# antonilo/unsupervised_detection

Hardware: AMD Instinct MI355X
Metric: frame-pairs/sec per adversarial step, DAVIS 480p batch4, 1/2/4/8 GPU (higher is better)
Workload: dtype f32

## Files before the change

### include/udet_debug.h

```cpp
#ifndef UDET_DEBUG_H
#define UDET_DEBUG_H
#include <stddef.h>
#ifdef __cplusplus
extern "C" {
#endif
void udet_debug_force_conv(int bm, int bn, int ks);
void udet_debug_conv_fp16(int on);
void udet_debug_force_wgrad(int nsplit, int dma);
int udet_debug_last_wgrad(void);
int udet_debug_last_wgrad_reduce(void);
int udet_debug_conv2d_backward_filter_ex(const float* x, int ldx, int x_coff, const float* dy, int ldy, int y_coff, const float* y_saved, int act,
                                         float alpha, const float* w, const float* b, const float* gamma, float bn_c, float* dw, float* db,
                                         float* dgamma, float* dbeta, int n, int h, int wd, int cin, int cout, int k, int stride, int dilation,
                                         int up, void* workspace, size_t workspace_bytes, void* stream);
void udet_debug_upb_min_pixels(long v);
void udet_debug_set_tuning(int on);
void udet_debug_force_pair(int on);
int udet_debug_last_pair(void);
int udet_debug_conv2d_pair(const float* xa, const float* xb, const float* wa, const float* wb, const float* ba, const float* bb, float* ya, float* yb,
                           int na, int nb, int h, int w, int cin, int cout, int k, int stride, int dilation, int act, float alpha, void* workspace,
                           size_t workspace_bytes, void* stream);
int udet_debug_last_conv(void);
#ifdef __cplusplus
}
#endif
#endif
```

### unsupervised_detection_amd/_devel.py

```python
from __future__ import annotations

import ctypes
import os

from ._ffi import lib as _lib

_PATH = os.path.join(os.path.dirname(os.path.abspath(__file__)), "libudet_debug.so")
if not os.path.exists(_PATH):
    raise RuntimeError(f"{_PATH} is missing: build it with `make -C unsupervised_detection_amd/csrc`")
dbg = ctypes.CDLL(_PATH, mode=ctypes.RTLD_GLOBAL)
dbg.udet_debug_force_conv.restype = None
dbg.udet_debug_force_conv.argtypes = [ctypes.c_int, ctypes.c_int, ctypes.c_int]
dbg.udet_debug_last_conv.restype = ctypes.c_int
dbg.udet_debug_last_conv.argtypes = []
dbg.udet_debug_conv_fp16.restype = None
dbg.udet_debug_conv_fp16.argtypes = [ctypes.c_int]
dbg.udet_debug_force_wgrad.restype = None
dbg.udet_debug_force_wgrad.argtypes = [ctypes.c_int, ctypes.c_int]
dbg.udet_debug_upb_min_pixels.restype = None
dbg.udet_debug_upb_min_pixels.argtypes = [ctypes.c_long]
dbg.udet_debug_set_tuning.restype = None
dbg.udet_debug_set_tuning.argtypes = [ctypes.c_int]
dbg.udet_debug_last_wgrad.restype = ctypes.c_int
dbg.udet_debug_last_wgrad.argtypes = []
dbg.udet_debug_force_pair.restype = None
dbg.udet_debug_force_pair.argtypes = [ctypes.c_int]
dbg.udet_debug_last_pair.restype = ctypes.c_int
dbg.udet_debug_last_pair.argtypes = []
dbg.udet_debug_conv2d_pair.restype = ctypes.c_int
dbg.udet_debug_conv2d_pair.argtypes = [ctypes.c_void_p] * 8 + [ctypes.c_int] * 10 + [ctypes.c_float, ctypes.c_void_p, ctypes.c_size_t, ctypes.c_void_p]
dbg.udet_debug_last_wgrad_reduce.restype = ctypes.c_int
dbg.udet_debug_last_wgrad_reduce.argtypes = []
_p, _i, _f = ctypes.c_void_p, ctypes.c_int, ctypes.c_float
dbg.udet_debug_conv2d_backward_filter_ex.restype = ctypes.c_int
dbg.udet_debug_conv2d_backward_filter_ex.argtypes = ([_p, _i, _i, _p, _i, _i, _p, _i, _f, _p, _p, _p, _f, _p, _p, _p, _p] + [_i] * 9
                                                     + [_p, ctypes.c_size_t, _p])
```

### unsupervised_detection_amd/csrc/conv_host.h

```cpp
#pragma once
#include "common.h"
namespace udet {
void same_pad(int in, int k, int s, int d, int* before, int* out);
void conv_setup_fwd(ConvParams& p, int N, int H, int W, int kh, int kw, int s, int d);
int conv_dgrad_classes(int s, int H, int W);
void conv_force_config(int bm, int bn, int ks);
bool conv_thin_n_ok(const ConvParams& p);
bool conv_thin_k_ok(const ConvParams& p);
int launch_conv_thin_n(const ConvParams& p, hipStream_t stream);
int launch_conv_thin_k(const ConvParams& p, hipStream_t stream);
bool conv_wino_geometry(const ConvParams& p, int* dil, int widx_at[9]);
bool conv_wino_ok(const ConvParams& p);
bool conv_wino_variant_ok(const ConvParams& p, int variant);
int conv_wino_np(int cout);
size_t conv_wino_floats(int Kc, int cout);
long conv_wino_workgroups(const ConvParams& p, int variant);
int conv_wino_max_ksplit(const ConvParams& p, int variant);
int launch_conv_wino(ConvParams& p, int variant, int ks, hipStream_t stream);
int launch_splitk_second_pass(const ConvParams& p, hipStream_t stream);
int launch_wino_pack(const float* src, float* dst, int R, int C, int Kc, int np, int k_split, int k_gap, int transposed, hipStream_t stream);
int launch_wino_from_packed(const ConvParams& p, float* dst, int np, hipStream_t stream);
void conv_debug_f16(int on);
int conv_debug_f16_on();
int conv_last_config();
void conv_set_tuning(int on);
int tuned_shapes();
void tune_dump(FILE* f);
bool tune_put_line(const char* line);
int conv_tune_rejected();
void wgrad_set_tuning(int on);
bool wgrad_wino_ok(const WgradParams& p);
int wgrad_wino_slices(const WgradParams& p, int wanted);
int launch_wgrad_wino(const WgradParams& q, int slices, int ldn, hipStream_t stream);
int wgrad_last_config();
enum { WGRAD_RED_FUSED_BN = 1 << 26, WGRAD_RED_SEPARATE_BN = 1 << 27, WGRAD_RED_SWAPPED = 1 << 28, WGRAD_RED_CLASSES = 1 << 29 };
int wgrad_last_reduce();
void setup_up_fwd(ConvParams& p, int N, int H, int W);
void wgrad_force(int nsplit, int dma);
void conv_force_pair(int on);
int conv_last_pair();
#define UDET_TUNE_ABI 6
bool conv_setup_dgrad(ConvParams& p, int cls, int N, int H, int W, int kh, int kw, int s, int d);
int launch_pack_weights(const float* src, float* dst, int T, int R, int C, int Kc, int ldw, int k_split, int k_gap,
                        int mode, const float* scale, hipStream_t stream);
int launch_pack_taps_into_n(const float* src, float* dst, int T, int R, int C, int Kc, int ldz, int k_split, int k_gap,
                            int transposed, hipStream_t stream);
int launch_pack_jobs(const PackJob* jobs_dev, int njobs, const float* wsrc, float* ws, float bn_c, hipStream_t stream);
int launch_fold_bn(const float* b, const float* gamma, const float* beta, float c, float* scale, float* bias_f, int n,
                   hipStream_t stream);
int launch_copy_channels(const float* src, int lds, int s_coff, float* dst, int ldd, int d_coff, long P, int C, float mul,
                         float add, hipStream_t stream);
int launch_warp(const float* img, const float* flow, int ldf, int f_coff, float flow_scale, float* out, int N, int H,
                int W, int C, int* dbg_idx, float* dbg_alpha, hipStream_t stream);
int launch_cost_volume(const float* c1, const float* wr, float* out, int ldo, int o_coff, int N, int H, int W, int C,
                       hipStream_t stream);
int launch_warp_cost_volume(const float* c1, const float* c2, const float* flow, int ldf, int f_coff, float flow_scale, float* out,
                            int ldo, int corr_coff, int c1_coff, float* warped_dbg, int N, int H, int W, int C, hipStream_t stream);
inline int round_up(int v, int m) { return (v + m - 1) / m * m; }
}
```

### unsupervised_detection_amd/csrc/conv_tile.hip

```cpp
#include <type_traits>

#include "common.h"
#include "conv_epilogue.h"

namespace udet {

typedef float floatx16 __attribute__((ext_vector_type(16)));
typedef _Float16 halfx4 __attribute__((ext_vector_type(4)));

__device__ __forceinline__ void tile_epilogue(const ConvParams& p, int off, int n, float v) {
  if (p.bias) v += p.bias[n];
  v = act_fwd(v, p.act, p.alpha);
  if (p.y2) p.y2[(size_t)off * p.ldy2 + p.y2_coff + n] = v;
  if (p.res) v += p.res[(size_t)off * p.ldres + p.res_coff + n];
  float* dst = p.y + (size_t)off * p.ldy + p.y_coff + n;
  if (p.accumulate) v += *dst;
  *dst = v;
  if (p.uo && n >= p.u_c0 && n < p.u_c1)
    p.uo[(size_t)off * p.ldu + p.u_coff + n] = v * act_dfo(p.ua[(size_t)off * p.ldua + p.ua_coff + n], p.uact, p.ualpha);
}

struct TileGeom {
  int min_dy, min_dx, PH, PW;
};
struct TileGeoms {
  TileGeom g[4];
  int cb;
};

typedef float floatx4 __attribute__((ext_vector_type(4)));
#define TILE_MT_BIG 16
#define TILE_MW_BIG 3
#define TILE_MT_SMALL 8
#define TILE_MW_SMALL 2
template <int NW> struct TileAcc;
template <> struct TileAcc<32> { floatx16 v; };
template <> struct TileAcc<16> { floatx4 v[2]; };

template <int TH, int NW, int TILE_MT, int TILE_MW, bool F16 = false>
__global__ __launch_bounds__(256) void conv_tile_kernel(const ConvParams p, const TileGeoms gs) {
  constexpr int TW = 32;
  constexpr int TM = TH / 4;
  constexpr int NG = 64 / NW;
  constexpr int NQ4 = NW / 4;
  extern __shared__ __attribute__((aligned(16))) float4 smem4[];
  const int cls = blockIdx.z;
  const TileGeom g = gs.g[cls];
  const int tap0 = p.cls_tap[cls], ntc = p.cls_tap[cls + 1] - tap0;
  const int ooy = p.ncls > 1 ? (cls >> 1) : p.ooy, oox = p.ncls > 1 ? (cls & 1) : p.oox;
  const int PIX = g.PH * g.PW;
  const int PIXP = PIX | 1;
  const int CB = p.Kc < gs.cb ? p.Kc : gs.cb;
  const int CQB = CB >> 2;
  float4* T4 = smem4;
  float4* W4 = smem4 + (size_t)CQB * PIXP;
  int* tapoff = reinterpret_cast<int*>(W4 + ((size_t)ntc * CQB + NG) * NW);
  int* pixoff = tapoff + ntc;
  int* qoff = pixoff + PIX;

  const int t = threadIdx.x, lane = t & 63, wave = t >> 6;
  const int col = lane & (NW - 1), grp = lane / NW;
  const int tiles_x = (p.OWq + TW - 1) / TW, tiles_y = (p.OHq + TH - 1) / TH;
  const int bid = blockIdx.x;
  const int tx = bid % tiles_x, ty = (bid / tiles_x) % tiles_y, n = bid / (tiles_x * tiles_y);
  const int oy0 = ty * TH, ox0 = tx * TW;
  const int n0 = blockIdx.y * NW;
  const int iy0 = oy0 * p.isy + g.min_dy, ix0 = ox0 * p.isx + g.min_dx;
  const int Hs = p.H >> p.up_shift, Ws = p.W >> p.up_shift;
  const float* xb = p.x + (size_t)n * Hs * Ws * p.ldx + p.x_coff;

  for (int i = t; i < ntc; i += 256) tapoff[i] = (p.taps[tap0 + i].dy - g.min_dy) * g.PW + (p.taps[tap0 + i].dx - g.min_dx);
  for (int pix = t; pix < PIX; pix += 256) {
    const int py = pix / g.PW, px = pix - py * g.PW;
    const int iy = iy0 + py, ix = ix0 + px;
    int o = -1;
    if ((unsigned)iy < (unsigned)p.H && (unsigned)ix < (unsigned)p.W) o = ((iy >> p.up_shift) * Ws + (ix >> p.up_shift)) * p.ldx;
    pixoff[pix] = o;
  }

  TileAcc<NW> acc[TM];
#pragma unroll
  for (int i = 0; i < TM; ++i) {
    if constexpr (NW == 32) {
#pragma unroll
      for (int r = 0; r < 16; ++r) acc[i].v[r] = 0.f;
    } else {
#pragma unroll
      for (int h = 0; h < 2; ++h)
#pragma unroll
        for (int r = 0; r < 4; ++r) acc[i].v[h][r] = 0.f;
    }
  }
  int abase[TM];
#pragma unroll
  for (int i = 0; i < TM; ++i) abase[i] = ((wave * TM + i) * p.isy) * g.PW + col * p.isx;
  const int ahalf = 16 * p.isx;
  const float xscale = F16 ? p.f16_xscale : 1.f;

  float4 tv[TILE_MT];
  float4 wv[TILE_MW][4];
  auto fetch = [&](int c0, int cw) {
    const int cq = cw >> 2, NQ = ntc * cq;
    const int cq_shift = (cq & (cq - 1)) == 0 ? __builtin_ctz(cq) : -1;
#pragma unroll
    for (int u = 0; u < TILE_MT; ++u) {
      const int e = t + u * 256;
      tv[u] = make_float4(0.f, 0.f, 0.f, 0.f);
      if (e < PIX * cq) {
        const int pix = cq_shift >= 0 ? e >> cq_shift : e / cq, c4 = e - pix * cq;
        const int o = pixoff[pix];
        if (o >= 0) tv[u] = *reinterpret_cast<const float4*>(xb + (size_t)o + c0 + c4 * 4);
      }
    }
#pragma unroll
    for (int u = 0; u < TILE_MW; ++u) {
      const int e = t + u * 256;
      wv[u][0] = wv[u][1] = wv[u][2] = wv[u][3] = make_float4(0.f, 0.f, 0.f, 0.f);
      if (e < NQ * NQ4) {
        const int n4 = e % NQ4, q = e / NQ4;
        const int tap = cq_shift >= 0 ? q >> cq_shift : q / cq, c4 = q - tap * cq;
        const int nn = n0 + n4 * 4;
        if (nn < p.ldw) {
          const float* src = p.wp + ((size_t)p.taps[tap0 + tap].widx * p.Kc + c0 + c4 * 4) * p.ldw + nn;
          wv[u][0] = *reinterpret_cast<const float4*>(src);
          wv[u][1] = *reinterpret_cast<const float4*>(src + p.ldw);
          wv[u][2] = *reinterpret_cast<const float4*>(src + 2 * (size_t)p.ldw);
          wv[u][3] = *reinterpret_cast<const float4*>(src + 3 * (size_t)p.ldw);
        }
      }
    }
  };
  auto commit = [&](int cw) {
    const int cq = cw >> 2, NQ = ntc * cq;
    const int cq_shift = (cq & (cq - 1)) == 0 ? __builtin_ctz(cq) : -1;
#pragma unroll
    for (int u = 0; u < TILE_MT; ++u) {
      const int e = t + u * 256;
      if (e < PIX * cq) {
        const int pix = cq_shift >= 0 ? e >> cq_shift : e / cq, c4 = e - pix * cq;
        T4[(size_t)c4 * PIXP + pix] = tv[u];
      }
    }
#pragma unroll
    for (int u = 0; u < TILE_MW; ++u) {
      const int e = t + u * 256;
      if (e < NQ * NQ4) {
        const int n4 = e % NQ4, q = e / NQ4;
        float4* d = W4 + (size_t)q * NW + n4 * 4;
        d[0] = make_float4(wv[u][0].x, wv[u][1].x, wv[u][2].x, wv[u][3].x);
        d[1] = make_float4(wv[u][0].y, wv[u][1].y, wv[u][2].y, wv[u][3].y);
        d[2] = make_float4(wv[u][0].z, wv[u][1].z, wv[u][2].z, wv[u][3].z);
        d[3] = make_float4(wv[u][0].w, wv[u][1].w, wv[u][2].w, wv[u][3].w);
      }
    }
    for (int e = t; e < NG * NW; e += 256) W4[(size_t)NQ * NW + e] = make_float4(0.f, 0.f, 0.f, 0.f);
    for (int q = t; q < NQ + 3 * NG; q += 256) {
      int o = 0;
      if (q < NQ) {
        const int tap = cq_shift >= 0 ? q >> cq_shift : q / cq, c4 = q - tap * cq;
        o = c4 * PIXP + tapoff[tap];
      }
      qoff[q] = o;
    }
  };

  for (int c0 = -CB; c0 < p.Kc; c0 += CB) {
    const int cw = c0 < 0 ? CB : (p.Kc - c0 < CB ? p.Kc - c0 : CB);
    const int cq = cw >> 2, NQ = ntc * cq;
    __syncthreads();
    if (c0 >= 0) {
      commit(cw);
      __syncthreads();
    }
    if (c0 + CB < p.Kc) fetch(c0 + CB, p.Kc - (c0 + CB) < CB ? p.Kc - (c0 + CB) : CB);
    if (c0 < 0) continue;

    constexpr int NA = NW == 32 ? TM : 2 * TM;
    const int steps = (NQ + NG - 1) / NG;
    int q = grp;
    int off1 = qoff[q + NG];
    float4 b = W4[(size_t)q * NW + col];
    float4 a[NA];
    {
      const float4* ta = T4 + qoff[q];
#pragma unroll
      for (int i = 0; i < TM; ++i) {
        if constexpr (NW == 32) {
          a[i] = ta[abase[i]];
        } else {
          a[2 * i] = ta[abase[i]];
          a[2 * i + 1] = ta[abase[i] + ahalf];
        }
      }
    }
    for (int j = 0; j < steps; ++j) {
      float4 bn = b, an[NA];
#pragma unroll
      for (int i = 0; i < NA; ++i) an[i] = a[i];
      int off2 = 0;
      if (j + 1 < steps) {
        q += NG;
        off2 = qoff[q + NG];
        bn = W4[(size_t)q * NW + col];
        const float4* ta = T4 + off1;
#pragma unroll
        for (int i = 0; i < TM; ++i) {
          if constexpr (NW == 32) {
            an[i] = ta[abase[i]];
// ... 15 lines not shown
            for (int h = 0; h < 2; ++h) {
              const float4 av = a[2 * i + h];
              const halfx4 ah = halfx4{(_Float16)(av.x * xscale), (_Float16)(av.y * xscale), (_Float16)(av.z * xscale), (_Float16)(av.w * xscale)};
              acc[i].v[h] = __builtin_amdgcn_mfma_f32_16x16x16f16(ah, bh, acc[i].v[h], 0, 0, 0);
            }
          }
        }
      } else
#pragma unroll
      for (int i = 0; i < TM; ++i) {
        if constexpr (NW == 32) {
          acc[i].v = __builtin_amdgcn_mfma_f32_32x32x2f32(a[i].x, b.x, acc[i].v, 0, 0, 0);
          acc[i].v = __builtin_amdgcn_mfma_f32_32x32x2f32(a[i].y, b.y, acc[i].v, 0, 0, 0);
          acc[i].v = __builtin_amdgcn_mfma_f32_32x32x2f32(a[i].z, b.z, acc[i].v, 0, 0, 0);
          acc[i].v = __builtin_amdgcn_mfma_f32_32x32x2f32(a[i].w, b.w, acc[i].v, 0, 0, 0);
        } else {
          acc[i].v[0] = __builtin_amdgcn_mfma_f32_16x16x4f32(a[2 * i].x, b.x, acc[i].v[0], 0, 0, 0);
          acc[i].v[1] = __builtin_amdgcn_mfma_f32_16x16x4f32(a[2 * i + 1].x, b.x, acc[i].v[1], 0, 0, 0);
          acc[i].v[0] = __builtin_amdgcn_mfma_f32_16x16x4f32(a[2 * i].y, b.y, acc[i].v[0], 0, 0, 0);
          acc[i].v[1] = __builtin_amdgcn_mfma_f32_16x16x4f32(a[2 * i + 1].y, b.y, acc[i].v[1], 0, 0, 0);
          acc[i].v[0] = __builtin_amdgcn_mfma_f32_16x16x4f32(a[2 * i].z, b.z, acc[i].v[0], 0, 0, 0);
          acc[i].v[1] = __builtin_amdgcn_mfma_f32_16x16x4f32(a[2 * i + 1].z, b.z, acc[i].v[1], 0, 0, 0);
          acc[i].v[0] = __builtin_amdgcn_mfma_f32_16x16x4f32(a[2 * i].w, b.w, acc[i].v[0], 0, 0, 0);
          acc[i].v[1] = __builtin_amdgcn_mfma_f32_16x16x4f32(a[2 * i + 1].w, b.w, acc[i].v[1], 0, 0, 0);
        }
      }
      __builtin_amdgcn_sched_group_barrier(0x100, NA + 2, 0);
      if constexpr (!F16) __builtin_amdgcn_sched_group_barrier(0x008, 4 * NA, 0);
      b = bn;
#pragma unroll
      for (int i = 0; i < NA; ++i) a[i] = an[i];
      off1 = off2;
    }
  }

  if (F16 && xscale != 1.f) {
    const float inv = 1.f / xscale;
#pragma unroll
    for (int i = 0; i < TM; ++i) {
      if constexpr (NW == 32) {
#pragma unroll
        for (int r = 0; r < 16; ++r) acc[i].v[r] *= inv;
      } else {
#pragma unroll
        for (int h = 0; h < 2; ++h)
#pragma unroll
          for (int r = 0; r < 4; ++r) acc[i].v[h][r] *= inv;
      }
    }
  }
  const int nn = n0 + col;
  if (nn >= p.Cout) return;
  const bool plain = !p.y2 && !p.res && !p.accumulate && !p.uo;
  const float bias = p.bias ? p.bias[nn] : 0.f;
  auto rows = [&](auto&& emit) {
#pragma unroll
    for (int i = 0; i < TM; ++i) {
      const int oy = oy0 + wave * TM + i;
      if (oy >= p.OHq) continue;
      const int row = (n * p.OH + oy * p.osy + ooy) * p.OW + oox;
      if constexpr (NW == 32) {
#pragma unroll
        for (int r = 0; r < 16; ++r) {
          const int ox = ox0 + (r & 3) + 8 * (r >> 2) + 4 * grp;
          if (ox < p.OWq) emit(row, ox, acc[i].v[r]);
        }
      } else {
#pragma unroll
        for (int h = 0; h < 2; ++h)
#pragma unroll
          for (int r = 0; r < 4; ++r) {
            const int ox = ox0 + h * 16 + grp * 4 + r;
            if (ox < p.OWq) emit(row, ox, acc[i].v[h][r]);
          }
      }
    }
  };
  const EpiAct ea = epi_act(p);
  if (plain) {
    float* ycol = p.y + p.y_coff + nn;
    const int xstep = p.osx * p.ldy;
    if (p.act == ACT_ELU) rows([&](int row, int ox, float v) { ycol[(size_t)row * p.ldy + (size_t)ox * xstep] = act_fwd_c<true>(v + bias, ea.slope); });
    else rows([&](int row, int ox, float v) { ycol[(size_t)row * p.ldy + (size_t)ox * xstep] = act_fwd_c<false>(v + bias, ea.slope); });
    return;
  }
  const bool emit_u = p.uo && nn >= p.u_c0 && nn < p.u_c1;
  auto generic = [&](auto ELU) {
#pragma unroll
    for (int i = 0; i < TM; ++i) {
      const int oy = oy0 + wave * TM + i;
      if (oy >= p.OHq) continue;
      const int row = (n * p.OH + oy * p.osy + ooy) * p.OW + oox;
      constexpr int NE = NW == 32 ? 16 : 8;
      float rs[NE], ac[NE], ua[NE];
      int off[NE];
#pragma unroll
      for (int e = 0; e < NE; ++e) {
        const int ox = NW == 32 ? ox0 + (e & 3) + 8 * (e >> 2) + 4 * grp : ox0 + (e >> 2) * 16 + grp * 4 + (e & 3);
        off[e] = ox < p.OWq ? row + ox * p.osx : -1;
        rs[e] = ac[e] = ua[e] = 0.f;
        if (off[e] >= 0) {
          if (p.res) rs[e] = p.res[(size_t)off[e] * p.ldres + p.res_coff + nn];
          if (p.accumulate) ac[e] = p.y[(size_t)off[e] * p.ldy + p.y_coff + nn];
          if (emit_u) ua[e] = p.ua[(size_t)off[e] * p.ldua + p.ua_coff + nn];
        }
      }
#pragma unroll
      for (int e = 0; e < NE; ++e) {
        if (off[e] < 0) continue;
        float v;
        if constexpr (NW == 32) v = acc[i].v[e];
        else v = acc[i].v[e >> 2][e & 3];
        v = act_fwd_c<decltype(ELU)::value>(v + bias, ea.slope);
        if (p.y2) p.y2[(size_t)off[e] * p.ldy2 + p.y2_coff + nn] = v;
        if (p.res) v += rs[e];
        if (p.accumulate) v += ac[e];
        p.y[(size_t)off[e] * p.ldy + p.y_coff + nn] = v;
        if (emit_u) p.uo[(size_t)off[e] * p.ldu + p.u_coff + nn] = v * act_dfo_c(ua[e], ea);
      }
    }
  };
  if (p.act == ACT_ELU) generic(std::true_type());
  else generic(std::false_type());
}

size_t conv_tile_lds_bytes(const ConvParams& p, int th, int cbmax, TileGeoms* gout, bool* big) {
  if (big) *big = false;
  if (p.ntaps < 1 || p.xa != nullptr || p.Kc % 4 != 0 || p.isy != p.isx || p.isy < 1 || p.isy > 2) return 0;
  const int ncls = p.ncls > 1 ? p.ncls : 1;
  if (ncls > 4) return 0;
  if (cbmax != 32 && cbmax != 16) return 0;
  if (gout) gout->cb = cbmax;
  const size_t cb = p.Kc < cbmax ? p.Kc : cbmax;
  size_t worst = 0;
  for (int c = 0; c < ncls; ++c) {
    const int t0 = ncls > 1 ? p.cls_tap[c] : 0, t1 = ncls > 1 ? p.cls_tap[c + 1] : p.ntaps;
    int mn_y = 0, mx_y = 0, mn_x = 0, mx_x = 0;
    for (int t = t0; t < t1; ++t) {
      if (t == t0 || p.taps[t].dy < mn_y) mn_y = p.taps[t].dy;
      if (t == t0 || p.taps[t].dy > mx_y) mx_y = p.taps[t].dy;
      if (t == t0 || p.taps[t].dx < mn_x) mn_x = p.taps[t].dx;
      if (t == t0 || p.taps[t].dx > mx_x) mx_x = p.taps[t].dx;
    }
    TileGeom g;
    g.min_dy = mn_y; g.min_dx = mn_x;
    g.PH = (th - 1) * p.isy + (mx_y - mn_y) + 1;
    g.PW = 31 * p.isx + (mx_x - mn_x) + 1;
    if (gout) gout->g[c] = g;
    const size_t pix = (size_t)g.PH * g.PW, ntc = (size_t)(t1 - t0), cqb = cb / 4, nw = p.Cout <= 16 ? 16 : 32;
    const size_t ng = 64 / nw;
    const size_t bytes = (cqb * (pix | 1) + (ntc * cqb + ng) * nw) * 16 + (ntc + pix + ntc * cqb + 3 * ng + 8) * sizeof(float);
    if (pix * cqb > 256 * TILE_MT_BIG || ntc * cqb * (nw / 4) > 256 * TILE_MW_BIG) return 0;
    if (big && (pix * cqb > 256 * TILE_MT_SMALL || ntc * cqb * (nw / 4) > 256 * TILE_MW_SMALL)) *big = true;
    worst = bytes > worst ? bytes : worst;
  }
  return worst;
}

int launch_conv_tile(const ConvParams& p, int th, int cbmax, hipStream_t stream) {
  TileGeoms g;
  bool big = false;
  const size_t lds = conv_tile_lds_bytes(p, th, cbmax, &g, &big);
  if (lds == 0 || lds > 96 * 1024 || (th != 8 && th != 4)) {
    set_error("conv_tile: launch not eligible");
    return UDET_ERR_UNSUPPORTED;
  }
  typedef void (*Kern)(const ConvParams, const TileGeoms);
  static const Kern K[2][2][2] = {
      {{conv_tile_kernel<8, 32, TILE_MT_SMALL, TILE_MW_SMALL>, conv_tile_kernel<8, 32, TILE_MT_BIG, TILE_MW_BIG>},
       {conv_tile_kernel<8, 16, TILE_MT_SMALL, TILE_MW_SMALL>, conv_tile_kernel<8, 16, TILE_MT_BIG, TILE_MW_BIG>}},
      {{conv_tile_kernel<4, 32, TILE_MT_SMALL, TILE_MW_SMALL>, conv_tile_kernel<4, 32, TILE_MT_BIG, TILE_MW_BIG>},
       {conv_tile_kernel<4, 16, TILE_MT_SMALL, TILE_MW_SMALL>, conv_tile_kernel<4, 16, TILE_MT_BIG, TILE_MW_BIG>}}};
  static bool attr_set = false;
  if (!attr_set) {
    for (int a = 0; a < 2; ++a)
      for (int b = 0; b < 2; ++b)
        for (int c = 0; c < 2; ++c)
          (void)hipFuncSetAttribute(reinterpret_cast<const void*>(K[a][b][c]), hipFuncAttributeMaxDynamicSharedMemorySize, 96 * 1024);
    attr_set = true;
  }
  const int tiles = ((p.OWq + 31) / 32) * ((p.OHq + th - 1) / th) * p.N;
  const int ncls = p.ncls > 1 ? p.ncls : 1;
  const bool n16 = p.Cout <= 16;
  dim3 grid(tiles, n16 ? 1 : (p.Cout + 31) / 32, ncls);
  if (p.f16) {
    static const Kern K16[2][2][2] = {
        {{conv_tile_kernel<8, 32, TILE_MT_SMALL, TILE_MW_SMALL, true>, conv_tile_kernel<8, 32, TILE_MT_BIG, TILE_MW_BIG, true>},
         {conv_tile_kernel<8, 16, TILE_MT_SMALL, TILE_MW_SMALL, true>, conv_tile_kernel<8, 16, TILE_MT_BIG, TILE_MW_BIG, true>}},
        {{conv_tile_kernel<4, 32, TILE_MT_SMALL, TILE_MW_SMALL, true>, conv_tile_kernel<4, 32, TILE_MT_BIG, TILE_MW_BIG, true>},
         {conv_tile_kernel<4, 16, TILE_MT_SMALL, TILE_MW_SMALL, true>, conv_tile_kernel<4, 16, TILE_MT_BIG, TILE_MW_BIG, true>}}};
    static bool attr16 = false;
    if (!attr16) {
      for (int a = 0; a < 2; ++a)
        for (int b = 0; b < 2; ++b)
          for (int c = 0; c < 2; ++c)
            (void)hipFuncSetAttribute(reinterpret_cast<const void*>(K16[a][b][c]), hipFuncAttributeMaxDynamicSharedMemorySize, 96 * 1024);
      attr16 = true;
    }
    UDET_LAUNCH(K16[th == 4][n16][big], grid, dim3(256), lds, stream, p, g);
  } else {
    UDET_LAUNCH(K[th == 4][n16][big], grid, dim3(256), lds, stream, p, g);
  }
  UDET_HIP(hipGetLastError());
  return UDET_OK;
}

}
```

### unsupervised_detection_amd/csrc/devel/api_debug.hip

```cpp
#include <string.h>

#include "../../../include/udet_debug.h"
#include "../conv_host.h"
#include "../plan.h"

using namespace udet;

extern "C" {
int udet_debug_last_conv(void) { return conv_last_config(); }
void udet_debug_force_conv(int bm, int bn, int ks) { conv_force_config(bm, bn, ks); }
void udet_debug_conv_fp16(int on) { conv_debug_f16(on); }
void udet_debug_force_wgrad(int nsplit, int dma) { wgrad_force(nsplit, dma); }
int udet_debug_last_wgrad(void) { return wgrad_last_config(); }
int udet_debug_last_wgrad_reduce(void) { return wgrad_last_reduce(); }
int udet_debug_conv2d_backward_filter_ex(const float* x, int ldx, int x_coff, const float* dy, int ldy, int y_coff, const float* y_saved, int act,
                                         float alpha, const float* w, const float* b, const float* gamma, float bn_c, float* dw, float* db,
                                         float* dgamma, float* dbeta, int n, int h, int wd, int cin, int cout, int k, int stride, int dilation,
                                         int up, void* workspace, size_t workspace_bytes, void* stream_) {
  hipStream_t stream = (hipStream_t)stream_;
  if (!x || !dy || !dw || n < 1 || h < 1 || wd < 1 || cin < 1 || cout < 1 || k < 1 || k * k > UDET_MAX_TAPS || dilation < 1 ||
      (stride != 1 && stride != 2) || up < 0 || up > 2) {
    set_error("debug_backward_filter_ex: bad argument");
    return UDET_ERR_ARG;
  }
// ... 12 lines not shown
  if (up == 2 && (!gamma || y_saved || k != 3 || stride != 1 || dilation != 1)) {
    set_error("debug_backward_filter_ex: the class-structured form is a BN-folded 3x3 stride-1 layer on dU");
    return UDET_ERR_ARG;
  }
  if (!workspace || (reinterpret_cast<uintptr_t>(workspace) & 63) || workspace_bytes < 128 * sizeof(float)) {
    set_error("debug_backward_filter_ex: workspace must be 64-byte aligned and hold the zero block");
    return UDET_ERR_ARG;
  }
  float* zero = reinterpret_cast<float*>(workspace);
  const int us = up ? 1 : 0;
  WgradParams p;
  memset(&p, 0, sizeof(p));
  p.x = x; p.ldx = ldx; p.x_coff = x_coff; p.N = n; p.Cin = cin;
  p.dy = dy; p.ldy = ldy; p.y_coff = y_coff; p.Cout = cout;
  if (y_saved && act != UDET_ACT_NONE) { p.ya = y_saved; p.yact = act; p.yalpha = alpha; }
  p.dw = dw; p.db = db;
  p.partial = zero + 64; p.partial_floats = workspace_bytes / sizeof(float) - 64;
  p.zero16 = zero;
  if (gamma) { p.w = w; p.b = b; p.gamma = gamma; p.dgamma = dgamma; p.dbeta = dbeta; p.bn_c = bn_c; }
  ConvParams g;
  memset(&g, 0, sizeof(g));
  conv_setup_fwd(g, n, h << us, wd << us, k, k, stride, dilation);
  p.H = h << us; p.W = wd << us; p.up_shift = us;
  p.OH = g.OH; p.OW = g.OW; p.isy = p.isx = stride;
  p.ntaps = g.ntaps;
  memcpy(p.taps, g.taps, sizeof(g.taps));
  UDET_HIP(hipMemsetAsync(zero, 0, 64 * sizeof(float), stream));
  if (up == 2) return launch_wgrad_up_T(p, h, wd, stream);
  return launch_wgrad_T(p, k * k, stream);
}
void udet_debug_upb_min_pixels(long v) { plan_debug_upb_min_pixels(v); }
void udet_debug_force_pair(int on) { conv_force_pair(on); }
int udet_debug_last_pair(void) { return conv_last_pair(); }
int udet_debug_conv2d_pair(const float* xa, const float* xb, const float* wa, const float* wb, const float* ba, const float* bb, float* ya, float* yb,
                           int na, int nb, int h, int w, int cin, int cout, int k, int stride, int dilation, int act, float alpha, void* workspace,
                           size_t workspace_bytes, void* stream_) {
  hipStream_t stream = (hipStream_t)stream_;
  if (cin % 8 != 0 || k * k > UDET_MAX_TAPS) { set_error("debug_conv2d_pair: cin must be a multiple of 8"); return UDET_ERR_SHAPE; }
  const int kc = cin, ldw = round_up(cout, 4);
  const size_t wfl = ((size_t)k * k * kc * ldw + 63) & ~(size_t)63, part_fl = (size_t)4 << 20, zero_fl = 64 + UDET_MAX_TICKETS;
  if (workspace_bytes < (2 * wfl + part_fl + zero_fl) * sizeof(float)) { set_error("debug_conv2d_pair: workspace too small"); return UDET_ERR_ARG; }
  float* wpa = reinterpret_cast<float*>(workspace);
  float* wpb = wpa + wfl;
  float* part = wpb + wfl;
  float* zero = part + part_fl;
  UDET_HIP(hipMemsetAsync(zero, 0, zero_fl * sizeof(float), stream));
  UDET_TRY(launch_pack_weights(wa, wpa, k * k, cin, cout, kc, ldw, kc, 0, 0, nullptr, stream));
  UDET_TRY(launch_pack_weights(wb, wpb, k * k, cin, cout, kc, ldw, kc, 0, 0, nullptr, stream));
  ConvParams p[2];
  for (int i = 0; i < 2; ++i) {
    memset(&p[i], 0, sizeof(ConvParams));
    conv_setup_fwd(p[i], i ? nb : na, h, w, k, k, stride, dilation);
    p[i].x = i ? xb : xa; p[i].ldx = cin; p[i].wp = i ? wpb : wpa; p[i].Kc = kc; p[i].ldw = ldw; p[i].bias = i ? bb : ba;
    p[i].y = i ? yb : ya; p[i].ldy = cout; p[i].Cout = cout; p[i].act = act; p[i].alpha = alpha;
    p[i].partial = part; p[i].partial_cap = part_fl; p[i].zero16 = zero; p[i].tickets = reinterpret_cast<int*>(zero + 64);
  }
  return launch_conv_pair(p[0], p[1], stream);
}
void udet_debug_set_tuning(int on) {
  conv_set_tuning(on);
  wgrad_set_tuning(on);
}
}
```

Baseline: 501.9.

## Make conv tile kernel persistent with cross-tile input prefetch and occupancy-sized grid

New measurement: 503.8 (median of 6 runs). About the same (+0.4%).

```diff
diff --git a/include/udet_debug.h b/include/udet_debug.h
--- a/include/udet_debug.h
+++ b/include/udet_debug.h
@@ -17,6 +17,7 @@
 void udet_debug_set_tuning(int on);
 void udet_debug_force_pair(int on);
 int udet_debug_last_pair(void);
+void udet_debug_tile_workgroups(int n);
 int udet_debug_conv2d_pair(const float* xa, const float* xb, const float* wa, const float* wb, const float* ba, const float* bb, float* ya, float* yb,
                            int na, int nb, int h, int w, int cin, int cout, int k, int stride, int dilation, int act, float alpha, void* workspace,
                            size_t workspace_bytes, void* stream);
diff --git a/unsupervised_detection_amd/_devel.py b/unsupervised_detection_amd/_devel.py
--- a/unsupervised_detection_amd/_devel.py
+++ b/unsupervised_detection_amd/_devel.py
@@ -27,6 +27,8 @@
 dbg.udet_debug_force_pair.argtypes = [ctypes.c_int]
 dbg.udet_debug_last_pair.restype = ctypes.c_int
 dbg.udet_debug_last_pair.argtypes = []
+dbg.udet_debug_tile_workgroups.restype = None
+dbg.udet_debug_tile_workgroups.argtypes = [ctypes.c_int]
 dbg.udet_debug_conv2d_pair.restype = ctypes.c_int
 dbg.udet_debug_conv2d_pair.argtypes = [ctypes.c_void_p] * 8 + [ctypes.c_int] * 10 + [ctypes.c_float, ctypes.c_void_p, ctypes.c_size_t, ctypes.c_void_p]
 dbg.udet_debug_last_wgrad_reduce.restype = ctypes.c_int
diff --git a/unsupervised_detection_amd/csrc/conv_host.h b/unsupervised_detection_amd/csrc/conv_host.h
--- a/unsupervised_detection_amd/csrc/conv_host.h
+++ b/unsupervised_detection_amd/csrc/conv_host.h
@@ -38,6 +38,7 @@
 void setup_up_fwd(ConvParams& p, int N, int H, int W);
 void wgrad_force(int nsplit, int dma);
 void conv_force_pair(int on);
+void conv_tile_workgroup_cap(int n);
 int conv_last_pair();
 #define UDET_TUNE_ABI 6
 bool conv_setup_dgrad(ConvParams& p, int cls, int N, int H, int W, int kh, int kw, int s, int d);
diff --git a/unsupervised_detection_amd/csrc/conv_tile.hip b/unsupervised_detection_amd/csrc/conv_tile.hip
--- a/unsupervised_detection_amd/csrc/conv_tile.hip
+++ b/unsupervised_detection_amd/csrc/conv_tile.hip
@@ -1,4 +1,8 @@
+#include <atomic>
+#include <map>
+#include <mutex>
 #include <type_traits>
+#include <utility>
 
 #include "common.h"
 #include "conv_epilogue.h"
@@ -37,13 +41,17 @@
 template <> struct TileAcc<32> { floatx16 v; };
 template <> struct TileAcc<16> { floatx4 v[2]; };
 
-template <int TH, int NW, int TILE_MT, int TILE_MW, bool F16 = false>
-__global__ __launch_bounds__(256) void conv_tile_kernel(const ConvParams p, const TileGeoms gs) {
+template <int TH, int NW, int TILE_MT, int TILE_MW, bool MULTI, bool F16 = false>
+__global__ __launch_bounds__(256, TILE_MT == TILE_MT_SMALL ? 3 : 2) void conv_tile_kernel(const ConvParams p, const TileGeoms gs) {
   constexpr int TW = 32;
   constexpr int TM = TH / 4;
   constexpr int NG = 64 / NW;
   constexpr int NQ4 = NW / 4;
+  constexpr bool XPREF = !MULTI && NW == 16;
   extern __shared__ __attribute__((aligned(16))) float4 smem4[];
+  const int tiles_x = (p.OWq + TW - 1) / TW, tiles_y = (p.OHq + TH - 1) / TH;
+  const int tiles = tiles_x * tiles_y * p.N;
+  if ((int)blockIdx.x >= tiles) return;
   const int cls = blockIdx.z;
   const TileGeom g = gs.g[cls];
   const int tap0 = p.cls_tap[cls], ntc = p.cls_tap[cls + 1] - tap0;
@@ -60,37 +68,45 @@
 
   const int t = threadIdx.x, lane = t & 63, wave = t >> 6;
   const int col = lane & (NW - 1), grp = lane / NW;
-  const int tiles_x = (p.OWq + TW - 1) / TW, tiles_y = (p.OHq + TH - 1) / TH;
-  const int bid = blockIdx.x;
-  const int tx = bid % tiles_x, ty = (bid / tiles_x) % tiles_y, n = bid / (tiles_x * tiles_y);
-  const int oy0 = ty * TH, ox0 = tx * TW;
   const int n0 = blockIdx.y * NW;
-  const int iy0 = oy0 * p.isy + g.min_dy, ix0 = ox0 * p.isx + g.min_dx;
   const int Hs = p.H >> p.up_shift, Ws = p.W >> p.up_shift;
-  const float* xb = p.x + (size_t)n * Hs * Ws * p.ldx + p.x_coff;
+  const size_t img = (size_t)Hs * Ws * p.ldx;
+  int tx = blockIdx.x % tiles_x, ty = (blockIdx.x / tiles_x) % tiles_y, n = blockIdx.x / (tiles_x * tiles_y);
+  const int gx = gridDim.x % tiles_x, gy = (gridDim.x / tiles_x) % tiles_y, gn = gridDim.x / (tiles_x * tiles_y);
 
   for (int i = t; i < ntc; i += 256) tapoff[i] = (p.taps[tap0 + i].dy - g.min_dy) * g.PW + (p.taps[tap0 + i].dx - g.min_dx);
-  for (int pix = t; pix < PIX; pix += 256) {
-    const int py = pix / g.PW, px = pix - py * g.PW;
-    const int iy = iy0 + py, ix = ix0 + px;
-    int o = -1;
-    if ((unsigned)iy < (unsigned)p.H && (unsigned)ix < (unsigned)p.W) o = ((iy >> p.up_shift) * Ws + (ix >> p.up_shift)) * p.ldx;
-    pixoff[pix] = o;
-  }
+  const int py_t = t / g.PW, px_t = t - py_t * g.PW;
+  const int py_d = 256 / g.PW, px_d = 256 - py_d * g.PW;
+  auto build_pixoff = [&](int txx, int tyy) {
+    const int iy0 = tyy * TH * p.isy + g.min_dy, ix0 = txx * TW * p.isx + g.min_dx;
+    int py = py_t, px = px_t;
+    for (int pix = t; pix < PIX; pix += 256) {
+      const int iy = iy0 + py, ix = ix0 + px;
+      int o = -1;
+      if ((unsigned)iy < (unsigned)p.H && (unsigned)ix < (unsigned)p.W) o = ((iy >> p.up_shift) * Ws + (ix >> p.up_shift)) * p.ldx;
+      pixoff[pix] = o;
+      px += px_d; py += py_d;
+      if (px >= g.PW) { px -= g.PW; ++py; }
+    }
+  };
+  build_pixoff(tx, ty);
 
   TileAcc<NW> acc[TM];
-#pragma unroll
-  for (int i = 0; i < TM; ++i) {
-    if constexpr (NW == 32) {
-#pragma unroll
-      for (int r = 0; r < 16; ++r) acc[i].v[r] = 0.f;
-    } else {
-#pragma unroll
-      for (int h = 0; h < 2; ++h)
-#pragma unroll
-        for (int r = 0; r < 4; ++r) acc[i].v[h][r] = 0.f;
-    }
-  }
+  auto zero_acc = [&]() {
+#pragma unroll
+    for (int i = 0; i < TM; ++i) {
+      if constexpr (NW == 32) {
+#pragma unroll
+        for (int r = 0; r < 16; ++r) acc[i].v[r] = 0.f;
+      } else {
+#pragma unroll
+        for (int h = 0; h < 2; ++h)
+#pragma unroll
+          for (int r = 0; r < 4; ++r) acc[i].v[h][r] = 0.f;
+      }
+    }
+  };
+  zero_acc();
   int abase[TM];
 #pragma unroll
   for (int i = 0; i < TM; ++i) abase[i] = ((wave * TM + i) * p.isy) * g.PW + col * p.isx;
@@ -98,63 +114,93 @@
   const float xscale = F16 ? p.f16_xscale : 1.f;
 
   float4 tv[TILE_MT];
-  float4 wv[TILE_MW][4];
-  auto fetch = [&](int c0, int cw) {
-    const int cq = cw >> 2, NQ = ntc * cq;
-    const int cq_shift = (cq & (cq - 1)) == 0 ? __builtin_ctz(cq) : -1;
+  int tmap[MULTI ? 1 : TILE_MT];
+  const int cqb_shift = (CQB & (CQB - 1)) == 0 ? __builtin_ctz(CQB) : -1;
+  if constexpr (!MULTI) {
 #pragma unroll
     for (int u = 0; u < TILE_MT; ++u) {
       const int e = t + u * 256;
+      const int pix = cqb_shift >= 0 ? e >> cqb_shift : e / CQB, c4 = e - pix * CQB;
+      tmap[u] = e < PIX * CQB ? (pix | c4 << 16) : -1;
+    }
+  }
+  auto t_item = [&](int u, int& pix, int& c4) {
+    if constexpr (MULTI) {
+      int e = t + u * 256;
+      asm volatile("" : "+v"(e));
+      pix = e >> cqb_shift;
+      c4 = e < PIX * CQB ? e & (CQB - 1) : -1;
+    } else {
+      int m = tmap[u];
+      asm volatile("" : "+v"(m));
+      pix = m & 0xffff;
+      c4 = m >> 16;
+    }
+  };
+  auto fetch_t = [&](const float* xb, int c0, int cq) {
+#pragma unroll
+    for (int u = 0; u < TILE_MT; ++u) {
       tv[u] = make_float4(0.f, 0.f, 0.f, 0.f);
-      if (e < PIX * cq) {
-        const int pix = cq_shift >= 0 ? e >> cq_shift : e / cq, c4 = e - pix * cq;
+      int pix, c4;
+      t_item(u, pix, c4);
+      if ((unsigned)c4 < (unsigned)cq) {
         const int o = pixoff[pix];
         if (o >= 0) tv[u] = *reinterpret_cast<const float4*>(xb + (size_t)o + c0 + c4 * 4);
       }
     }
+  };
+  auto commit_t = [&](int cq) {
+#pragma unroll
+    for (int u = 0; u < TILE_MT; ++u) {
+      int pix, c4;
+      t_item(u, pix, c4);
+      if ((unsigned)c4 < (unsigned)cq) T4[c4 * PIXP + pix] = tv[u];
+    }
+  };
+  float4 wv[TILE_MW][4];
+  auto w_item = [&](int u, int& tap, int& c4, int& n4) {
+    int e = t + u * 256;
+    asm volatile("" : "+v"(e));
+    n4 = e % NQ4;
+    const int q = e / NQ4;
+    tap = cqb_shift >= 0 ? q >> cqb_shift : q / CQB;
+    c4 = e < ntc * CQB * NQ4 ? q - tap * CQB : -1;
+  };
+  auto fetch_w = [&](int c0, int cq) {
 #pragma unroll
     for (int u = 0; u < TILE_MW; ++u) {
-      const int e = t + u * 256;
       wv[u][0] = wv[u][1] = wv[u][2] = wv[u][3] = make_float4(0.f, 0.f, 0.f, 0.f);
-      if (e < NQ * NQ4) {
-        const int n4 = e % NQ4, q = e / NQ4;
-        const int tap = cq_shift >= 0 ? q >> cq_shift : q / cq, c4 = q - tap * cq;
-        const int nn = n0 + n4 * 4;
-        if (nn < p.ldw) {
-          const float* src = p.wp + ((size_t)p.taps[tap0 + tap].widx * p.Kc + c0 + c4 * 4) * p.ldw + nn;
-          wv[u][0] = *reinterpret_cast<const float4*>(src);
-          wv[u][1] = *reinterpret_cast<const float4*>(src + p.ldw);
-          wv[u][2] = *reinterpret_cast<const float4*>(src + 2 * (size_t)p.ldw);
-          wv[u][3] = *reinterpret_cast<const float4*>(src + 3 * (size_t)p.ldw);
-        }
-      }
-    }
-  };
-  auto commit = [&](int cw) {
-    const int cq = cw >> 2, NQ = ntc * cq;
+      int tap, c4, n4;
+      w_item(u, tap, c4, n4);
+      const int nn = n0 + n4 * 4;
+      if ((unsigned)c4 < (unsigned)cq && nn < p.ldw) {
+        const float* src = p.wp + ((size_t)p.taps[tap0 + tap].widx * p.Kc + c0 + c4 * 4) * p.ldw + nn;
+        wv[u][0] = *reinterpret_cast<const float4*>(src);
+        wv[u][1] = *reinterpret_cast<const float4*>(src + p.ldw);
+        wv[u][2] = *reinterpret_cast<const float4*>(src + 2 * (size_t)p.ldw);
+        wv[u][3] = *reinterpret_cast<const float4*>(src + 3 * (size_t)p.ldw);
+      }
+    }
+  };
+  auto commit_w = [&](int cq) {
+    const int NQ = ntc * cq;
     const int cq_shift = (cq & (cq - 1)) == 0 ? __builtin_ctz(cq) : -1;
 #pragma unroll
-    for (int u = 0; u < TILE_MT; ++u) {
-      const int e = t + u * 256;
-      if (e < PIX * cq) {
-        const int pix = cq_shift >= 0 ? e >> cq_shift : e / cq, c4 = e - pix * cq;
-        T4[(size_t)c4 * PIXP + pix] = tv[u];
-      }
-    }
-#pragma unroll
     for (int u = 0; u < TILE_MW; ++u) {
-      const int e = t + u * 256;
-      if (e < NQ * NQ4) {
-        const int n4 = e % NQ4, q = e / NQ4;
-        float4* d = W4 + (size_t)q * NW + n4 * 4;
+      int tap, c4, n4;
+      w_item(u, tap, c4, n4);
+      if ((unsigned)c4 < (unsigned)cq) {
+        float4* d = W4 + (size_t)(tap * cq + c4) * NW + n4 * 4;
         d[0] = make_float4(wv[u][0].x, wv[u][1].x, wv[u][2].x, wv[u][3].x);
         d[1] = make_float4(wv[u][0].y, wv[u][1].y, wv[u][2].y, wv[u][3].y);
         d[2] = make_float4(wv[u][0].z, wv[u][1].z, wv[u][2].z, wv[u][3].z);
         d[3] = make_float4(wv[u][0].w, wv[u][1].w, wv[u][2].w, wv[u][3].w);
       }
     }
-    for (int e = t; e < NG * NW; e += 256) W4[(size_t)NQ * NW + e] = make_float4(0.f, 0.f, 0.f, 0.f);
-    for (int q = t; q < NQ + 3 * NG; q += 256) {
+    int t_o = t;
+    asm volatile("" : "+v"(t_o));
+    for (int e = t_o; e < NG * NW; e += 256) W4[(size_t)NQ * NW + e] = make_float4(0.f, 0.f, 0.f, 0.f);
+    for (int q = t_o; q < NQ + 3 * NG; q += 256) {
       int o = 0;
       if (q < NQ) {
         const int tap = cq_shift >= 0 ? q >> cq_shift : q / cq, c4 = q - tap * cq;
@@ -164,16 +210,136 @@
     }
   };
 
-  for (int c0 = -CB; c0 < p.Kc; c0 += CB) {
-    const int cw = c0 < 0 ? CB : (p.Kc - c0 < CB ? p.Kc - c0 : CB);
+  const int nn = n0 + col;
+  const bool plain = !p.y2 && !p.res && !p.accumulate && !p.uo;
+  const float bias = p.bias && nn < p.Cout ? p.bias[nn] : 0.f;
+  const EpiAct ea = epi_act(p);
+  const bool emit_u = p.uo && nn >= p.u_c0 && nn < p.u_c1;
+  auto epilogue = [&]() {
+    if (F16 && xscale != 1.f) {
+      const float inv = 1.f / xscale;
+#pragma unroll
+      for (int i = 0; i < TM; ++i) {
+        if constexpr (NW == 32) {
+#pragma unroll
+          for (int r = 0; r < 16; ++r) acc[i].v[r] *= inv;
+        } else {
+#pragma unroll
+          for (int h = 0; h < 2; ++h)
+#pragma unroll
+            for (int r = 0; r < 4; ++r) acc[i].v[h][r] *= inv;
+        }
+      }
+    }
+    int grp_o = grp, nn_o = nn;
+    asm volatile("" : "+v"(grp_o), "+v"(nn_o));
+    if (nn_o >= p.Cout) return;
+    const int oy0 = ty * TH, ox0 = tx * TW;
+    auto rows = [&](auto&& emit) {
+#pragma unroll
+      for (int i = 0; i < TM; ++i) {
+        const int oy = oy0 + wave * TM + i;
+        if (oy >= p.OHq) continue;
+        const int row = (n * p.OH + oy * p.osy + ooy) * p.OW + oox;
+        if constexpr (NW == 32) {
+#pragma unroll
+          for (int r = 0; r < 16; ++r) {
+            const int ox = ox0 + (r & 3) + 8 * (r >> 2) + 4 * grp_o;
+            if (ox < p.OWq) emit(row, ox, acc[i].v[r]);
+          }
+        } else {
+#pragma unroll
+          for (int h = 0; h < 2; ++h)
+#pragma unroll
+            for (int r = 0; r < 4; ++r) {
+              const int ox = ox0 + h * 16 + grp_o * 4 + r;
+              if (ox < p.OWq) emit(row, ox, acc[i].v[h][r]);
+            }
+        }
+      }
+    };
+    if (plain) {
+      float* ycol = p.y + p.y_coff + nn_o;
+      const int xstep = p.osx * p.ldy;
+      if (p.act == ACT_ELU) rows([&](int row, int ox, float v) { ycol[(size_t)row * p.ldy + (size_t)ox * xstep] = act_fwd_c<true>(v + bias, ea.slope); });
+      else rows([&](int row, int ox, float v) { ycol[(size_t)row * p.ldy + (size_t)ox * xstep] = act_fwd_c<false>(v + bias, ea.slope); });
+      return;
+    }
+    auto generic = [&](auto ELU) {
+#pragma unroll
+      for (int i = 0; i < TM; ++i) {
+        const int oy = oy0 + wave * TM + i;
+        if (oy >= p.OHq) continue;
+        const int row = (n * p.OH + oy * p.osy + ooy) * p.OW + oox;
+        constexpr int NR = NW == 32 ? 16 : 8, NE = MULTI && NW == 32 ? 4 : NR;
+#pragma unroll
+        for (int e0 = 0; e0 < NR; e0 += NE) {
+          float rs[NE], ac[NE], ua[NE];
+          int off[NE];
+#pragma unroll
+          for (int k = 0; k < NE; ++k) {
+            const int e = e0 + k;
+            const int ox = NW == 32 ? ox0 + (e & 3) + 8 * (e >> 2) + 4 * grp_o : ox0 + (e >> 2) * 16 + grp_o * 4 + (e & 3);
+            off[k] = ox < p.OWq ? row + ox * p.osx : -1;
+            rs[k] = ac[k] = ua[k] = 0.f;
+            if (off[k] >= 0) {
+              if (p.res) rs[k] = p.res[(size_t)off[k] * p.ldres + p.res_coff + nn_o];
+              if (p.accumulate) ac[k] = p.y[(size_t)off[k] * p.ldy + p.y_coff + nn_o];
+              if (emit_u) ua[k] = p.ua[(size_t)off[k] * p.ldua + p.ua_coff + nn_o];
+            }
+          }
+#pragma unroll
+          for (int k = 0; k < NE; ++k) {
+            if (off[k] < 0) continue;
+            const int e = e0 + k;
+            float v;
+            if constexpr (NW == 32) v = acc[i].v[e];
+            else v = acc[i].v[e >> 2][e & 3];
+            v = act_fwd_c<decltype(ELU)::value>(v + bias, ea.slope);
+            if (p.y2) p.y2[(size_t)off[k] * p.ldy2 + p.y2_coff + nn_o] = v;
+            if (p.res) v += rs[k];
+            if (p.accumulate) v += ac[k];
+            p.y[(size_t)off[k] * p.ldy + p.y_coff + nn_o] = v;
+            if (emit_u) p.uo[(size_t)off[k] * p.ldu + p.u_coff + nn_o] = v * act_dfo_c(ua[k], ea);
+          }
+        }
+      }
+    };
+    if (p.act == ACT_ELU) generic(std::true_type());
+    else generic(std::false_type());
+  };
+
+  __syncthreads();
+  fetch_t(p.x + p.x_coff + (size_t)n * img, 0, CQB);
+  fetch_w(0, CQB);
+  if constexpr (!MULTI) commit_w(CQB);
+
+  for (int c0 = 0;;) {
+    const int cw = p.Kc - c0 < CB ? p.Kc - c0 : CB;
     const int cq = cw >> 2, NQ = ntc * cq;
+    const bool last_pass = !MULTI || c0 + CB >= p.Kc;
+    int ntx = tx, nty = ty, nn_img = n;
+    bool more = true;
     __syncthreads();
-    if (c0 >= 0) {
-      commit(cw);
-      __syncthreads();
-    }
-    if (c0 + CB < p.Kc) fetch(c0 + CB, p.Kc - (c0 + CB) < CB ? p.Kc - (c0 + CB) : CB);
-    if (c0 < 0) continue;
+    commit_t(cq);
+    if constexpr (MULTI) commit_w(cq);
+    if (last_pass) {
+      ntx += gx; nty += gy; nn_img += gn;
+      if (ntx >= tiles_x) { ntx -= tiles_x; ++nty; }
+      if (nty >= tiles_y) { nty -= tiles_y; ++nn_img; }
+      more = nn_img < p.N;
+      if (more) build_pixoff(ntx, nty);
+    }
+    __syncthreads();
+    const int nc0 = last_pass ? 0 : c0 + CB;
+    auto fetch_next = [&]() {
+      const int ncw = p.Kc - nc0 < CB ? p.Kc - nc0 : CB;
+      fetch_t(p.x + p.x_coff + (size_t)nn_img * img, nc0, ncw >> 2);
+      if constexpr (MULTI) fetch_w(nc0, ncw >> 2);
+    };
+    if constexpr (XPREF || MULTI) {
+      if (more && (XPREF || !last_pass)) fetch_next();
+    }
 
     constexpr int NA = NW == 32 ? TM : 2 * TM;
     const int steps = (NQ + NG - 1) / NG;
@@ -255,97 +421,18 @@
       for (int i = 0; i < NA; ++i) a[i] = an[i];
       off1 = off2;
     }
+    if (!last_pass) {
+      c0 += CB;
+      continue;
+    }
+    epilogue();
+    if (!more) break;
+    if constexpr (!XPREF) fetch_next();
+    zero_acc();
+    tx = ntx; ty = nty; n = nn_img; c0 = 0;
   }
-
-  if (F16 && xscale != 1.f) {
-    const float inv = 1.f / xscale;
-#pragma unroll
-    for (int i = 0; i < TM; ++i) {
-      if constexpr (NW == 32) {
-#pragma unroll
-        for (int r = 0; r < 16; ++r) acc[i].v[r] *= inv;
-      } else {
-#pragma unroll
-        for (int h = 0; h < 2; ++h)
-#pragma unroll
-          for (int r = 0; r < 4; ++r) acc[i].v[h][r] *= inv;
-      }
-    }
-  }
-  const int nn = n0 + col;
-  if (nn >= p.Cout) return;
-  const bool plain = !p.y2 && !p.res && !p.accumulate && !p.uo;
-  const float bias = p.bias ? p.bias[nn] : 0.f;
-  auto rows = [&](auto&& emit) {
-#pragma unroll
-    for (int i = 0; i < TM; ++i) {
-      const int oy = oy0 + wave * TM + i;
-      if (oy >= p.OHq) continue;
-      const int row = (n * p.OH + oy * p.osy + ooy) * p.OW + oox;
-      if constexpr (NW == 32) {
-#pragma unroll
-        for (int r = 0; r < 16; ++r) {
-          const int ox = ox0 + (r & 3) + 8 * (r >> 2) + 4 * grp;
-          if (ox < p.OWq) emit(row, ox, acc[i].v[r]);
-        }
-      } else {
-#pragma unroll
-        for (int h = 0; h < 2; ++h)
-#pragma unroll
-          for (int r = 0; r < 4; ++r) {
-            const int ox = ox0 + h * 16 + grp * 4 + r;
-            if (ox < p.OWq) emit(row, ox, acc[i].v[h][r]);
-          }
-      }
-    }
-  };
-  const EpiAct ea = epi_act(p);
-  if (plain) {
-    float* ycol = p.y + p.y_coff + nn;
-    const int xstep = p.osx * p.ldy;
-    if (p.act == ACT_ELU) rows([&](int row, int ox, float v) { ycol[(size_t)row * p.ldy + (size_t)ox * xstep] = act_fwd_c<true>(v + bias, ea.slope); });
-    else rows([&](int row, int ox, float v) { ycol[(size_t)row * p.ldy + (size_t)ox * xstep] = act_fwd_c<false>(v + bias, ea.slope); });
-    return;
-  }
-  const bool emit_u = p.uo && nn >= p.u_c0 && nn < p.u_c1;
-  auto generic = [&](auto ELU) {
-#pragma unroll
-    for (int i = 0; i < TM; ++i) {
-      const int oy = oy0 + wave * TM + i;
-      if (oy >= p.OHq) continue;
-      const int row = (n * p.OH + oy * p.osy + ooy) * p.OW + oox;
-      constexpr int NE = NW == 32 ? 16 : 8;
-      float rs[NE], ac[NE], ua[NE];
-      int off[NE];
-#pragma unroll
-      for (int e = 0; e < NE; ++e) {
-        const int ox = NW == 32 ? ox0 + (e & 3) + 8 * (e >> 2) + 4 * grp : ox0 + (e >> 2) * 16 + grp * 4 + (e & 3);
-        off[e] = ox < p.OWq ? row + ox * p.osx : -1;
-        rs[e] = ac[e] = ua[e] = 0.f;
-        if (off[e] >= 0) {
-          if (p.res) rs[e] = p.res[(size_t)off[e] * p.ldres + p.res_coff + nn];
-          if (p.accumulate) ac[e] = p.y[(size_t)off[e] * p.ldy + p.y_coff + nn];
-          if (emit_u) ua[e] = p.ua[(size_t)off[e] * p.ldua + p.ua_coff + nn];
-        }
-      }
-#pragma unroll
-      for (int e = 0; e < NE; ++e) {
-        if (off[e] < 0) continue;
-        float v;
-        if constexpr (NW == 32) v = acc[i].v[e];
-        else v = acc[i].v[e >> 2][e & 3];
-        v = act_fwd_c<decltype(ELU)::value>(v + bias, ea.slope);
-        if (p.y2) p.y2[(size_t)off[e] * p.ldy2 + p.y2_coff + nn] = v;
-        if (p.res) v += rs[e];
-        if (p.accumulate) v += ac[e];
-        p.y[(size_t)off[e] * p.ldy + p.y_coff + nn] = v;
-        if (emit_u) p.uo[(size_t)off[e] * p.ldu + p.u_coff + nn] = v * act_dfo_c(ua[e], ea);
-      }
-    }
-  };
-  if (p.act == ACT_ELU) generic(std::true_type());
-  else generic(std::false_type());
-}
+}
+
 
 size_t conv_tile_lds_bytes(const ConvParams& p, int th, int cbmax, TileGeoms* gout, bool* big) {
   if (big) *big = false;
@@ -380,6 +467,35 @@
   return worst;
 }
 
+static std::atomic<int> g_tile_wg_cap{0};
+void conv_tile_workgroup_cap(int n) { g_tile_wg_cap = n > 0 ? n : 0; }
+
+namespace {
+typedef void (*TileKern)(const ConvParams, const TileGeoms);
+template <bool F16>
+TileKern tile_kernel(int i) {
+  static const TileKern K[16] = {
+      conv_tile_kernel<8, 32, TILE_MT_SMALL, TILE_MW_SMALL, false, F16>, conv_tile_kernel<4, 32, TILE_MT_SMALL, TILE_MW_SMALL, false, F16>,
+      conv_tile_kernel<8, 16, TILE_MT_SMALL, TILE_MW_SMALL, false, F16>, conv_tile_kernel<4, 16, TILE_MT_SMALL, TILE_MW_SMALL, false, F16>,
+      conv_tile_kernel<8, 32, TILE_MT_BIG, TILE_MW_BIG, false, F16>,     conv_tile_kernel<4, 32, TILE_MT_BIG, TILE_MW_BIG, false, F16>,
+      conv_tile_kernel<8, 16, TILE_MT_BIG, TILE_MW_BIG, false, F16>,     conv_tile_kernel<4, 16, TILE_MT_BIG, TILE_MW_BIG, false, F16>,
+      conv_tile_kernel<8, 32, TILE_MT_SMALL, TILE_MW_SMALL, true, F16>,  conv_tile_kernel<4, 32, TILE_MT_SMALL, TILE_MW_SMALL, true, F16>,
+      conv_tile_kernel<8, 16, TILE_MT_SMALL, TILE_MW_SMALL, true, F16>,  conv_tile_kernel<4, 16, TILE_MT_SMALL, TILE_MW_SMALL, true, F16>,
+      conv_tile_kernel<8, 32, TILE_MT_BIG, TILE_MW_BIG, true, F16>,      conv_tile_kernel<4, 32, TILE_MT_BIG, TILE_MW_BIG, true, F16>,
+      conv_tile_kernel<8, 16, TILE_MT_BIG, TILE_MW_BIG, true, F16>,      conv_tile_kernel<4, 16, TILE_MT_BIG, TILE_MW_BIG, true, F16>};
+  return K[i];
+}
+constexpr int TILE_MAXDEV = 64;
+struct TileDevice {
+  std::once_flag once;
+  hipError_t attr = hipSuccess;
+  int cus = 0;
+  std::mutex mu;
+  std::map<std::pair<int, size_t>, int> occ;
+};
+TileDevice g_tile_dev[TILE_MAXDEV];
+}
+
 int launch_conv_tile(const ConvParams& p, int th, int cbmax, hipStream_t stream) {
   TileGeoms g;
   bool big = false;
@@ -388,42 +504,50 @@
     set_error("conv_tile: launch not eligible");
     return UDET_ERR_UNSUPPORTED;
   }
-  typedef void (*Kern)(const ConvParams, const TileGeoms);
-  static const Kern K[2][2][2] = {
-      {{conv_tile_kernel<8, 32, TILE_MT_SMALL, TILE_MW_SMALL>, conv_tile_kernel<8, 32, TILE_MT_BIG, TILE_MW_BIG>},
-       {conv_tile_kernel<8, 16, TILE_MT_SMALL, TILE_MW_SMALL>, conv_tile_kernel<8, 16, TILE_MT_BIG, TILE_MW_BIG>}},
-      {{conv_tile_kernel<4, 32, TILE_MT_SMALL, TILE_MW_SMALL>, conv_tile_kernel<4, 32, TILE_MT_BIG, TILE_MW_BIG>},
-       {conv_tile_kernel<4, 16, TILE_MT_SMALL, TILE_MW_SMALL>, conv_tile_kernel<4, 16, TILE_MT_BIG, TILE_MW_BIG>}}};
-  static bool attr_set = false;
-  if (!attr_set) {
-    for (int a = 0; a < 2; ++a)
-      for (int b = 0; b < 2; ++b)
-        for (int c = 0; c < 2; ++c)
-          (void)hipFuncSetAttribute(reinterpret_cast<const void*>(K[a][b][c]), hipFuncAttributeMaxDynamicSharedMemorySize, 96 * 1024);
-    attr_set = true;
-  }
+  int dev = 0;
+  UDET_HIP(hipGetDevice(&dev));
+  if (dev < 0 || dev >= TILE_MAXDEV) { set_error("conv_tile: device ordinal %d out of range", dev); return UDET_ERR_ARG; }
+  TileDevice& D = g_tile_dev[dev];
+  std::call_once(D.once, [&]() {
+    for (int i = 0; i < 32 && D.attr == hipSuccess; ++i)
+      D.attr = hipFuncSetAttribute(reinterpret_cast<const void*>(i < 16 ? tile_kernel<false>(i) : tile_kernel<true>(i - 16)),
+                                   hipFuncAttributeMaxDynamicSharedMemorySize, 96 * 1024);
+    if (D.attr == hipSuccess) D.attr = hipDeviceGetAttribute(&D.cus, hipDeviceAttributeMultiprocessorCount, dev);
+  });
+  UDET_HIP(D.attr);
   const int tiles = ((p.OWq + 31) / 32) * ((p.OHq + th - 1) / th) * p.N;
   const int ncls = p.ncls > 1 ? p.ncls : 1;
   const bool n16 = p.Cout <= 16;
-  dim3 grid(tiles, n16 ? 1 : (p.Cout + 31) / 32, ncls);
-  if (p.f16) {
-    static const Kern K16[2][2][2] = {
-        {{conv_tile_kernel<8, 32, TILE_MT_SMALL, TILE_MW_SMALL, true>, conv_tile_kernel<8, 32, TILE_MT_BIG, TILE_MW_BIG, true>},
-         {conv_tile_kernel<8, 16, TILE_MT_SMALL, TILE_MW_SMALL, true>, conv_tile_kernel<8, 16, TILE_MT_BIG, TILE_MW_BIG, true>}},
-        {{conv_tile_kernel<4, 32, TILE_MT_SMALL, TILE_MW_SMALL, true>, conv_tile_kernel<4, 32, TILE_MT_BIG, TILE_MW_BIG, true>},
-         {conv_tile_kernel<4, 16, TILE_MT_SMALL, TILE_MW_SMALL, true>, conv_tile_kernel<4, 16, TILE_MT_BIG, TILE_MW_BIG, true>}}};
-    static bool attr16 = false;
-    if (!attr16) {
-      for (int a = 0; a < 2; ++a)
-        for (int b = 0; b < 2; ++b)
-          for (int c = 0; c < 2; ++c)
-            (void)hipFuncSetAttribute(reinterpret_cast<const void*>(K16[a][b][c]), hipFuncAttributeMaxDynamicSharedMemorySize, 96 * 1024);
-      attr16 = true;
-    }
-    UDET_LAUNCH(K16[th == 4][n16][big], grid, dim3(256), lds, stream, p, g);
-  } else {
-    UDET_LAUNCH(K[th == 4][n16][big], grid, dim3(256), lds, stream, p, g);
+  const int inst = (th == 4) | n16 << 1 | big << 2 | (p.Kc > cbmax) << 3;
+  const TileKern kern = p.f16 ? tile_kernel<true>(inst) : tile_kernel<false>(inst);
+  int occ = 0;
+  {
+    std::lock_guard<std::mutex> lock(D.mu);
+    const auto key = std::make_pair(inst | (p.f16 ? 16 : 0), lds);
+    auto it = D.occ.find(key);
+    if (it == D.occ.end()) {
+      int v = 0;
+      UDET_HIP(hipOccupancyMaxActiveBlocksPerMultiprocessor(&v, reinterpret_cast<const void*>(kern), 256, lds));
+      it = D.occ.emplace(key, v < 1 ? 1 : v).first;
+    }
+    occ = it->second;
   }
+  const int slices = (n16 ? 1 : (p.Cout + 31) / 32) * ncls;
+  int slots = occ * D.cus / slices;
+  if (slots < 1) slots = 1;
+  int wgs = tiles;
+  if (tiles > slots) {
+#ifdef UDET_TILE_POLICY_MIN
+    wgs = slots;
+#else
+    const int per = (tiles + slots - 1) / slots;
+    wgs = (tiles + per - 1) / per;
+#endif
+  }
+  const int cap = g_tile_wg_cap.load();
+  if (cap > 0 && wgs > cap) wgs = cap;
+  dim3 grid(wgs, n16 ? 1 : (p.Cout + 31) / 32, ncls);
+  UDET_LAUNCH(kern, grid, dim3(256), lds, stream, p, g);
   UDET_HIP(hipGetLastError());
   return UDET_OK;
 }
diff --git a/unsupervised_detection_amd/csrc/devel/api_debug.hip b/unsupervised_detection_amd/csrc/devel/api_debug.hip
--- a/unsupervised_detection_amd/csrc/devel/api_debug.hip
+++ b/unsupervised_detection_amd/csrc/devel/api_debug.hip
@@ -68,6 +68,7 @@
 void udet_debug_upb_min_pixels(long v) { plan_debug_upb_min_pixels(v); }
 void udet_debug_force_pair(int on) { conv_force_pair(on); }
 int udet_debug_last_pair(void) { return conv_last_pair(); }
+void udet_debug_tile_workgroups(int n) { conv_tile_workgroup_cap(n); }
 int udet_debug_conv2d_pair(const float* xa, const float* xb, const float* wa, const float* wb, const float* ba, const float* bb, float* ya, float* yb,
                            int na, int nb, int h, int w, int cin, int cout, int k, int stride, int dilation, int act, float alpha, void* workspace,
                            size_t workspace_bytes, void* stream_) {
```
